# dropbox/lepton

Hardware: AMD Instinct MI355X
Metric: encode+decode MB/s (JPEG bytes/sec), bit-exact round trip (higher is better)
Workload: dtype int16/u8 (integer coder, no floating point)

## Files before the change

### lepton_amd/csrc/lep_enc5.h

```cpp
#pragma once
#include "lep_v3.h"
#ifdef LEP5_DEBUG
#include <cstdio>
#endif

namespace lep5 {
using namespace lep3;

constexpr int kRows = 64, kClasses = 10;
constexpr int kPRows = 63 + 14;
constexpr int kStreams = 2 * kRows * kClasses;
WDEV int stream_id(int ci, int row, int k) { return (ci * kRows + row) * kClasses + k; }
constexpr int kCoefSlice = 12 * 11 + 10 + 1;
constexpr int kSignSlice = 48, kNzSlice = 6 * 32, kEdgeNzSlice = 8 * 12, kDcSlice = 17 * 11 + 10 + 1;
constexpr uint32_t kThreshWords = 2u * 256 * 8 * 128;

WDEV uint32_t coef_entry(uint32_t vlow, int nres, int len, int bsr, int k, int u) {
    return vlow | ((uint32_t)nres << 10) | ((uint32_t)len << 14) | ((uint32_t)bsr << 18) | ((uint32_t)k << 23) | ((uint32_t)u << 27);
}
WDEV int coef_units(int len, int nres) { return ((len < 11 ? len + 1 : 11) + nres + 3) >> 2; }
WDEV uint32_t thresh_entry(uint32_t tbits, int n, int pcls, int lt, int u) {
    return tbits | ((uint32_t)n << 10) | ((uint32_t)pcls << 14) | ((uint32_t)lt << 23) | ((uint32_t)u << 27);
}
constexpr int kKeyRec = 4, kNzRec = 8, kEnRec = 8, kDcRec = 24;
// ... 1353 lines not shown
        LEP5_XSYNC();
        if (MODE == kEmit && wave == 0) {
            LANES(l) if (l < 16) LEP5_WSH(this).cursor[stream_id(l >> 3, 63, l & 7)] = LEP5_WSH(this).tcur[l];
            LSYNC();
            LANES(l) {
                for (int i = l; i < kStreams; i += 64)
                    for (uint32_t j = LEP5_WSH(this).cursor[i]; j < pl->base[i + 1]; ++j) gst(units() + j, 0u);
            }
        }
        return 0;
    }
};


constexpr int kCountWords = kStreams + 5;
WDEV void plan_segment(const uint32_t* counts, SegPlan5* P) {
    uint32_t at = 0;
    for (int i = 0; i < kStreams; ++i) { P->base[i] = at; P->cnt[i] = counts[i]; at += (counts[i] + 3u) & ~3u; }
    P->base[kStreams] = at;
    uint32_t bytes = at * 4;
    P->sign_cnt[0] = counts[kStreams]; P->sign_cnt[1] = counts[kStreams + 1];
    P->sign_base[0] = bytes; bytes += (P->sign_cnt[0] + 15u) & ~15u;
    P->sign_base[1] = bytes; bytes += (P->sign_cnt[1] + 15u) & ~15u;
    P->nblocks = counts[kStreams + 2];
    P->key_base = bytes; bytes += ((P->nblocks * (uint32_t)kKeyRec) + 15u) & ~15u;
    P->nz_base = bytes; bytes += P->nblocks * (uint32_t)kNzRec;
    P->en_base = bytes; bytes += P->nblocks * (uint32_t)kEnRec;
    P->dc_base = bytes; bytes += P->nblocks * (uint32_t)kDcRec;
    P->cls_base = bytes; bytes += 2u * kNumCls * 4u;
    P->place_base = bytes; bytes += 4u * P->nblocks * 4u;
    bytes = (bytes + 15u) & ~15u;
    P->nzs_base = bytes; bytes += (P->nblocks + 4u * 20u) * (uint32_t)kNzRec;
    P->ens_base[0] = bytes; bytes += (P->nblocks + 4u * 16u) * 4u;
    P->ens_base[1] = bytes; bytes += (P->nblocks + 4u * 16u) * 4u;
    P->dcs_base = bytes; bytes += (P->nblocks + 4u * 12u) * (uint32_t)kDcRec;
    bytes = (bytes + 15u) & ~15u;
    P->ckpt_base = bytes; bytes += (uint32_t)(kMaxParts * sizeof(Ckpt5));
    P->wstate_base = bytes; bytes += 64u;
    bytes = (bytes + 255u) & ~255u;
    P->ntiles = counts[kStreams + 4];
    P->at_base = bytes; bytes += P->ntiles * (uint32_t)(kAtRows * 64 * 4);
    P->arena_bytes = (bytes + 255u) & ~255u;
    P->bins_cap = (counts[kStreams + 3] + 127u) & ~127u;
    P->nbins = 0; P->status = 0; P->arena_off = 0; P->bins_off = 0;
}
template <class W>
WDEV void export_counts(const W& w, const Walk5Shared* sh, uint32_t* counts) {
    LANES(l) {
        for (int i = l; i < kStreams; i += 64) counts[i] = sh->cursor[i];
        if (l == 0) { counts[kStreams] = w.sign_pos[0]; counts[kStreams + 1] = w.sign_pos[1]; counts[kStreams + 2] = w.ord0; counts[kStreams + 3] = w.nbins; counts[kStreams + 4] = w.tile_no; }
    }
}

}
```

### lepton_amd/csrc/lep_gpu.hip

```cpp
#include <hip/hip_runtime.h>

#include <algorithm>
#include <cstdio>
#include <cstdlib>
#include <cstring>
#include <mutex>
#include <string>
#include <vector>

#include "../../include/lepton_mi355x.h"
#include "lep_buffers.h"

#define LEP_DEV __device__ __forceinline__
#include "lep_core.h"
#include "lep_enc3.h"
#include "lep_dec4.h"
#include "lep_enc5.h"
#include "lep_huff.h"
#include "lep_huffdec.h"
#include "lep_huffdec_simt.h"
#include "lep_huff_simt.h"
#include "lep_huffprog.h"
#include "lep_huffprog_simt.h"
#include "lep_huffprogdec.h"
// ... 89 lines not shown
        if (d >= 2) {
            const lep4::DivBy m = lep4::DivBy::of((uint32_t)d);
            const int32_t k = (int32_t)(0x7fffffff / d);
            for (int32_t n : {0, 1, -1, d, d - 1, -d, -d + 1, k * d, k * d - 1, -(k * d), 0x7fffffff, (int32_t)0x80000000, (int32_t)(f * 0x01000193u ^ t * 0x9e3779b9u)})
                if (lep4::div_by(n, m.mul, m.shift) != n / d) atomicAdd(mismatches, 1u);
        }
    }
}

template <int WAVES, int SCMASK = LEP_DEC4_SCALAR>
__global__ __launch_bounds__(64, WAVES) void lep_decode_v4_kernel(const ImageDev* __restrict__ images, const SegDev* __restrict__ segs,
                                                           uint32_t* models, NSum* ns_area, const uint64_t* ns_offsets,
                                                           uint8_t* streams, uint32_t* stream_len, int32_t* status, uint32_t* bins) {
    __shared__ lep4::Dec4Shared sh;
    const int s = blockIdx.x, lane = threadIdx.x;
    const SegDev seg = segs[s];
    const ImageDev* img = images + seg.image;
    uint32_t* model = models + (size_t)s * kModelStride;
    NSum* ns = ns_area + ns_offsets[s];
    reset_segment_state<lep3::kModelWords>(model, ns, img->ns_total, lane);
    __syncthreads();
    lep4::Dec4WaveT<SCMASK> w;
#ifdef LEP_PROF
    w.prof_begin(&g_prof4[s & 8191][0]);
#endif
    int rc = w.run(img, seg, model, ns, &sh, streams + seg.stream_off, stream_len[seg.slot]);
#ifdef LEP_PROF
    w.prof_end();
#endif
    if (lane != 0) return;
    status[seg.slot] = rc;
    bins[seg.slot] = w.nbins;
}


template <int MODE, int NW>
__global__ __launch_bounds__(64 * NW) void lep_enc5_walk_kernel(const ImageDev* __restrict__ images, const SegDev* __restrict__ segs, NSum* ns_all,
                                                         const uint64_t* __restrict__ ns_off, lep5::SegPlan5* plans, uint8_t* arena, uint16_t* bins,
                                                         uint32_t* counts, int part, int nparts) {
    lep5::Walk5Shared* sh = reinterpret_cast<lep5::Walk5Shared*>(lep5::lep5_lds);
    const int s = blockIdx.x;
    const SegDev seg = segs[s];
    lep5::SegPlan5* P = plans + s;
    if (MODE == lep5::kGather && P->status) return;
    lep5::Walk5<MODE, NW> w;
    const int rc = w.run(images + seg.image, seg, ns_all + ns_off[s], sh, P, arena, bins, (int)(threadIdx.x >> 6), part, nparts);
    if (threadIdx.x >= 64) return;
    if (MODE == lep5::kCount) lep5::export_counts(w, sh, counts + (size_t)s * lep5::kCountWords);
    if (threadIdx.x == 0) {
        if (MODE == lep5::kEmit) P->status = rc;
        if (MODE == lep5::kGather && part + 1 == nparts) P->nbins = w.nbins;
    }
}
template <int PHASE>
__global__ __launch_bounds__(64) void lep_enc5_wchunk_kernel(const lep5::SegPlan5* __restrict__ plans, const uint16_t* __restrict__ bins, const SegDev* __restrict__ segs,
                                                         int nseg, int K, lep5::WChunk5* recs, uint8_t* streams, uint32_t* stream_len, int32_t* status, uint32_t* nbins_out) {
    const int id = (int)(blockIdx.x * 64 + threadIdx.x);
    if (PHASE == 0 || PHASE == 2) {
        const int seg = id / K, k = id - seg * K;
        if (seg >= nseg) return;
        if (PHASE == 2) __builtin_amdgcn_s_setprio(3);
        if (PHASE == 0) lep5::wchunk_range_lane(plans[seg], bins, recs + (size_t)seg * K + k, k, K);
        else lep5::wchunk_code_lane(plans[seg], bins, segs[seg], streams, recs + (size_t)seg * K + k, k, K);
    } else {
        if (id >= nseg) return;
        if (PHASE == 1) { status[segs[id].slot] = 0; nbins_out[segs[id].slot] = plans[id].nbins; lep5::wchunk_link_lane(plans[id], bins, recs + (size_t)id * K, K); }
        else lep5::wchunk_stitch_lane(plans[id], segs[id], streams, stream_len, status, recs + (size_t)id * K, K);
    }
}
__global__ void lep_enc5_plan_kernel(const uint32_t* __restrict__ counts, lep5::SegPlan5* plans, int nseg) {
    const int s = (int)(blockIdx.x * blockDim.x + threadIdx.x);
    if (s < nseg) lep5::plan_segment(counts + (size_t)s * lep5::kCountWords, plans + s);
}
__global__ __launch_bounds__(64) void lep_enc5_offsets_kernel(lep5::SegPlan5* plans, int nseg, uint64_t* totals) {
    uint64_t a = 0, b = 0;
    for (int s0 = 0; s0 < nseg; s0 += 64) {
        const int s = s0 + (int)threadIdx.x;
        const uint32_t ab = s < nseg ? plans[s].arena_bytes : 0u, bc = s < nseg ? plans[s].bins_cap : 0u;
        int oa, ob;
        const int va = (int)(ab >> 8), vb = (int)(bc >> 7);
        const int ta = lepwave::wave_excl_scan(&va, &oa), tb = lepwave::wave_excl_scan(&vb, &ob);
        if (s < nseg) { plans[s].arena_off = a + ((uint64_t)(uint32_t)oa << 8); plans[s].bins_off = b + ((uint64_t)(uint32_t)ob << 7); }
        a += (uint64_t)(uint32_t)ta << 8; b += (uint64_t)(uint32_t)tb << 7;
    }
    if (threadIdx.x == 0) { totals[0] = a; totals[1] = b; }
}
__global__ void lep_enc5_fill_kernel(uint4* p, size_t n16, uint32_t v) {
    const uint4 x = make_uint4(v, v, v, v);
    for (size_t i = blockIdx.x * (size_t)blockDim.x + threadIdx.x; i < n16; i += (size_t)gridDim.x * blockDim.x) p[i] = x;
}
__global__ __launch_bounds__(64) void lep_enc5_bucket_kernel(const lep5::SegPlan5* __restrict__ plans, uint8_t* arena) {
    __shared__ lep5::BucketShared sh;
    lep5::bucket_wave(plans + blockIdx.x, arena, &sh);
}
struct Fold5CoefShared { uint16_t slice[lep5::kCoefSlice * 64]; };
__global__ __launch_bounds__(64) void lep_enc5_fold_coef_kernel(const lep5::SegPlan5* __restrict__ plans, uint8_t* arena, int nseg, int groups) {
    __shared__ Fold5CoefShared shc;
    const int grp = (int)blockIdx.x % groups, job = (int)blockIdx.x / groups;
    const int ci = job / 630, row = (job % 630) / 10, k = job % 10;
    const int sid = lep5::stream_id(ci, row, k), seg = grp * 64 + (int)threadIdx.x;
    const bool work = seg < nseg && !plans[seg].status && plans[seg].cnt[sid] != 0;
    if (!__ballot(work)) return;
    lep5::fold_coef_wave(plans, arena, grp * 64, nseg, sid, reinterpret_cast<lep5::FoldShared*>(&shc));
}
struct Fold5SmallShared { uint16_t slice[lep5::kEdgeNzSlice * 64]; };
__global__ __launch_bounds__(64) void lep_enc5_fold_small_kernel(const lep5::SegPlan5* __restrict__ plans, uint8_t* arena, uint32_t* thresh_models, int nseg, int groups, int job0) {
// ... 172 lines not shown
    w.run_scan<true>(scans + k, &sh, rows, deps + k, progress, k);
}

__global__ __launch_bounds__(64, 8) void lep_huffman_decode_kernel(const lephuff::HuffDecImage* __restrict__ images, lephuff::HuffDecRow* rows) {
    __shared__ lephuff::HuffDecShared sh;
    __builtin_amdgcn_s_setprio(3);
    lephuff::HuffDecWave w;
    w.run(images + blockIdx.x, &sh, rows);
}

__global__ __launch_bounds__(64) void lep_huffman_simt_settle_kernel(const lephuff::HuffDecImage* __restrict__ images, lephuff::SimtImage* si, const lephuff::SimtWave* waves,
                                                                     const lephuff::SimtSub* in, lephuff::SimtSub* out, int settle) {
    __shared__ lephuff::SimtShared sh;
    const lephuff::SimtWave w = waves[blockIdx.x];
    lephuff::simt_guess_or_settle(images + w.image, &sh, si + w.image, in + si[w.image].first, out + si[w.image].first, w.first_sub, settle);
}
__global__ __launch_bounds__(64) void lep_huffman_simt_place_kernel(const lephuff::HuffDecImage* __restrict__ images, lephuff::SimtImage* si, const lephuff::SimtSub* sub,
                                                                    lephuff::SimtPlace* place, int passes, lephuff::HuffDecRow* rows) {
    const int i = (int)blockIdx.x;
    lephuff::simt_place(images + i, si + i, sub + si[i].first, place + si[i].first, passes, rows);
}
__global__ __launch_bounds__(64) void lep_huffman_simt_write_kernel(const lephuff::HuffDecImage* __restrict__ images, lephuff::SimtImage* si, const lephuff::SimtWave* waves,
                                                                    const lephuff::SimtSub* sub, const lephuff::SimtPlace* place, lephuff::HuffDecRow* rows) {
    __shared__ lephuff::SimtShared sh;
    __shared__ lephuff::SimtTile tile;
    const lephuff::SimtWave w = waves[blockIdx.x];
    lephuff::simt_write(images + w.image, &sh, &tile, si + w.image, sub + si[w.image].first, place + si[w.image].first, rows, w.first_sub);
}
__global__ void lep_huffman_simt_finish_kernel(const lephuff::HuffDecImage* __restrict__ images, int nimg, lephuff::HuffDecRow* rows, const lephuff::SimtImage* si) {
    const int i = (int)(blockIdx.x * blockDim.x + threadIdx.x);
    if (i >= nimg) return;
    lephuff::HuffDecRow* last = rows + images[i].rows_off + images[i].mcuv;
    int status = si[i].status & 0x3fffff;
    if (last->aux == lephuff::kHuffDecRowUnwritten) { status |= 2; last->aux = 255; }
    if (images[i].flags & lephuff::kHuffDecRstTable) {
        const int pad = lephuff::simt_intervals_pad(si + i, &status);
        last->aux = pad | (status << 8);
        return;
    }
    last->aux = (last->aux & (255 | lephuff::kHuffDecRowTruncated)) | (status << 8);
}

}

struct lep_gpu {
    int device = 0;
    hipStream_t stream = nullptr;
    hipEvent_t ev0 = nullptr, ev1 = nullptr;
    bool timed = false;
    bool released = false;
    int enc5_min = 8;
    hipStream_t stream2 = nullptr, stream3 = nullptr;
    hipEvent_t ev_fork = nullptr, ev_join = nullptr, ev_join3 = nullptr;
    int huffprog_pipeline = 1;
    int huffprog_split = 0;
    int huffprogdec_rst = 1;
    uint32_t huffprogdec_rst_floor = lephuff::kRstPieceFloor;
    int huffprogdec_win = 1;
    int huffprog_simt = 1;
    int huffprog_simt_rst = 1;
    uint32_t huffprog_forms[4] = {0, 0, 0, 0};
    int huffenc_simt = 1;
    int simt_sub_bits = 0;
    int huffprog_pipeline_max = 16384;
    int enc5_waves = 2;
    int enc5_parts = 8;
    hipEvent_t ev_part[8] = {nullptr, nullptr, nullptr, nullptr, nullptr, nullptr, nullptr, nullptr};
    long enc5_wlanes = 131072;
    int enc5_wmaxseg = 4096;
    int enc5_wchunks = 64;
    int enc5_gather_wgs = 0;
    int enc5_fold_apart = 0;
    size_t enc5_scratch_max = ~(size_t)0;
    hipEvent_t ev_stage[8] = {nullptr, nullptr, nullptr, nullptr, nullptr, nullptr, nullptr, nullptr};
    int nstage = 0;
    int enc_waves = 0;
    int enc_pair_max = 1280;
    int dec_company = 0;
    int dec_waves = 0;
    std::string err;
    const char* last_kernel = "";
    struct Vmm {
        bool on = false;
        size_t chunk = (size_t)512 << 20;
        hipMemAllocationProp prop;
        hipMemAccessDesc access;
        std::vector<hipMemGenericAllocationHandle_t> pool;
        size_t mapped_total = 0, creates = 0, releases = 0;
    } vmm;
    enum Ws {
        W_ENC5_ENTRIES,
        W_ENC5_BINLIST,
        W_MODELS, W_MODELS_1,
        W_NS, W_NS_1,
        W_TRIMMED,
        W_META = W_TRIMMED, W_META_1,
        W_ENC5_PLANS,
        W_ENC5_WCHUNKS,
        W_BLOCKS, W_STREAMS, W_LENS,
        W_HUFF, W_HUFF_1,
        W_HUFFENC, W_HUFFENC_1,
        W_HUFFPROG, W_HUFFPROG_1,
        W_HUFFPROGSIMT, W_HUFFPROGSIMT_1,
        W_HUFFSEQ, W_HUFFSEQ_1,
        W_HUFFPROGDEC,
        W_HUFFPROGRST,
        W_HUFFDEC,
        W_HUFFPAR,
        W_COUNT
    };
    lepbuf::DevBuf<> ws[W_COUNT];
    int cur = 0;
    hipEvent_t ev_enc5_done = nullptr;
    uint32_t* d_bins = nullptr;
    std::vector<uint32_t> h_bins;
    struct Staging { void* host = nullptr; size_t cap = 0; hipEvent_t ev = nullptr; bool used = false; };
    Staging staging[16];
    int staging_next = 0;
    std::vector<void*> staging_retired;
    lepbuf::PinBuf<char> h_huffprog[2];
    int huffprog_turn = 0;
};

#define HIPCHK(g, call)                                                                        \
// ... 74 lines not shown
    const size_t old = b.mapped;
    while (b.mapped < want) {
        hipMemGenericAllocationHandle_t h;
        if (!V.pool.empty()) { h = V.pool.back(); V.pool.pop_back(); --V.creates; }
        else if (hipMemCreate(&h, V.chunk, &V.prop, 0) != hipSuccess) {
            (void)hipGetLastError();
            if (may_release) { may_release = false; release_idle_caches(g); if (!V.pool.empty()) continue; }
            {
                while (b.mapped > old) { b.mapped -= V.chunk; (void)hipMemUnmap(b.va + b.mapped, V.chunk); V.pool.push_back(b.chunks.back()); b.chunks.pop_back(); V.mapped_total -= V.chunk; }
                g->err = "hipMemCreate: out of device memory";
                return LEP_GPU_ERROR;
            }
        }
        ++V.creates;
        if (hipMemMap(b.va + b.mapped, V.chunk, 0, h, 0) != hipSuccess) { (void)hipGetLastError(); (void)hipMemRelease(h); g->err = "hipMemMap failed"; return LEP_GPU_ERROR; }
        b.chunks.push_back(h); b.mapped += V.chunk; V.mapped_total += V.chunk;
    }
    if (b.mapped > old) HIPCHK(g, hipMemSetAccess(b.va + old, b.mapped - old, &V.access, 1));
    w.set(b.va, b.mapped);
    return 0;
}
static int ensure(lep_gpu* g, Workspace& w, size_t need, bool may_release = true) {
    if (w.cap >= need) return 0;
    if (g->vmm.on && (need >= ((size_t)32 << 20) || w.v.va)) {
        if (!w.v.va) HIPCHK(g, w.release());
        return vmm_ensure(g, w, need, may_release);
    }
    hipError_t e = w.ensure(need, need / 8);
    if (e != hipSuccess && may_release) {
        (void)hipGetLastError();
        release_idle_caches(g);
        e = w.ensure(need);
    }
    if (e != hipSuccess) { g->err = std::string("hipMalloc: ") + hipGetErrorString(e); return LEP_GPU_ERROR; }
    return 0;
}

#include "lep_derive.h"


constexpr int kEnc5NoMemory = -1000;
static int launch_enc5(lep_gpu* g, const ImageDev* d_img, const SegDev* d_seg, const uint64_t* d_nsoff, int nseg, uint8_t* d_streams,
                       uint32_t* d_stream_len, int32_t* d_status, hipStream_t st) {
    Workspace &models = g->ws[lep_gpu::W_MODELS + g->cur], &ns = g->ws[lep_gpu::W_NS + g->cur];
    Workspace &ws_plans = g->ws[lep_gpu::W_ENC5_PLANS], &ws_entries = g->ws[lep_gpu::W_ENC5_ENTRIES], &ws_binlist = g->ws[lep_gpu::W_ENC5_BINLIST], &wchunks = g->ws[lep_gpu::W_ENC5_WCHUNKS];
    if (!g->stream2) {
        HIPCHK(g, hipEventCreateWithFlags(&g->ev_enc5_done, hipEventDisableTiming));
        for (auto& e : g->ev_part) HIPCHK(g, hipEventCreateWithFlags(&e, hipEventDisableTiming));
        HIPCHK(g, hipStreamCreateWithFlags(&g->stream2, hipStreamNonBlocking));
        HIPCHK(g, hipStreamCreateWithFlags(&g->stream3, hipStreamNonBlocking));
        HIPCHK(g, hipEventCreateWithFlags(&g->ev_fork, hipEventDisableTiming));
        HIPCHK(g, hipEventCreateWithFlags(&g->ev_join, hipEventDisableTiming));
        HIPCHK(g, hipEventCreateWithFlags(&g->ev_join3, hipEventDisableTiming));
        for (auto& e : g->ev_stage) HIPCHK(g, hipEventCreate(&e));
    }
    lepbuf::Layout L;
    L.add<lep5::SegPlan5>((size_t)nseg);
    const size_t o_counts = L.add<uint32_t>((size_t)nseg * lep5::kCountWords), o_tot = L.add<uint64_t>(2);
    HIPCHK(g, hipStreamWaitEvent(st, g->ev_enc5_done, 0));
    if (int rc = ensure(g, ws_plans, L.padded())) return rc;
    lep5::SegPlan5* plans = ws_plans.at<lep5::SegPlan5>(0);
    uint32_t* counts = ws_plans.at<uint32_t>(o_counts);
    uint64_t* d_tot = ws_plans.at<uint64_t>(o_tot);
    const int groups = (nseg + 63) / 64;
    g->nstage = 0;
    HIPCHK(g, hipEventRecord(g->ev_stage[0], st));
    const bool two = g->enc5_waves == 2;
    const int nparts = std::min(std::max(g->enc5_parts, 1), (int)lep5::kMaxParts);
    auto walk = [&](int mode, uint8_t* entries, uint16_t* binlist, int part = 0) {
        size_t lds = lep5::walk_lds_bytes(mode);
        if (mode == lep5::kGather && g->enc5_gather_wgs > 0) lds = std::max(lds, (size_t)(160 * 1024 / g->enc5_gather_wgs) & ~(size_t)255);
#define LEP_WALK(MODE, NW) hipLaunchKernelGGL((lep_enc5_walk_kernel<MODE, NW>), dim3(nseg), dim3(64 * NW), lds, st, d_img, d_seg, (NSum*)ns.p, d_nsoff, plans, entries, binlist, counts, part, nparts)
        if (mode == lep5::kCount) { if (two) LEP_WALK(lep5::kCount, 2); else LEP_WALK(lep5::kCount, 1); }
        else if (mode == lep5::kEmit) { if (two) LEP_WALK(lep5::kEmit, 2); else LEP_WALK(lep5::kEmit, 1); }
        else { if (two) LEP_WALK(lep5::kGather, 2); else LEP_WALK(lep5::kGather, 1); }
#undef LEP_WALK
    };
    walk(lep5::kCount, nullptr, nullptr);
    hipLaunchKernelGGL(lep_enc5_plan_kernel, dim3(groups), dim3(64), 0, st, (const uint32_t*)counts, plans, nseg);
    hipLaunchKernelGGL(lep_enc5_offsets_kernel, dim3(1), dim3(64), 0, st, plans, nseg, d_tot);
    hipLaunchKernelGGL(lep_enc5_fill_kernel, dim3(4096), dim3(256), 0, st, (uint4*)models.p, (size_t)nseg * lep5::kThreshWords / 4, kBranchInit);
    uint64_t tot[2] = {0, 0};
    HIPCHK(g, hipMemcpyAsync(tot, d_tot, sizeof tot, hipMemcpyDeviceToHost, st));
    HIPCHK(g, hipStreamSynchronize(st));
    if ((size_t)tot[0] + (size_t)tot[1] * 2 > g->enc5_scratch_max || ensure(g, ws_entries, (size_t)tot[0] + 256, false) || ensure(g, ws_binlist, (size_t)tot[1] * 2 + 256, false)) {
        (void)hipGetLastError();
        g->err.clear();
        static bool told = false;
        if (!told) { told = true; fprintf(stderr, "lepton-mi355x: no room for the split-phase encoder's scratch (%.1f GB for %d segments): single-kernel encoder\n", ((double)tot[0] + 2.0 * (double)tot[1]) / 1e9, nseg); }
        return kEnc5NoMemory;
    }
    {
        HIPCHK(g, hipEventRecord(g->ev_stage[1], st));
        walk(lep5::kEmit, (uint8_t*)ws_entries.p, nullptr);
        HIPCHK(g, hipEventRecord(g->ev_stage[2], st));
        hipLaunchKernelGGL(lep_enc5_bucket_kernel, dim3(nseg), dim3(64), 0, st, (const lep5::SegPlan5*)plans, (uint8_t*)ws_entries.p);
        HIPCHK(g, hipEventRecord(g->ev_fork, st));
        HIPCHK(g, hipStreamWaitEvent(g->stream2, g->ev_fork, 0));
        HIPCHK(g, hipStreamWaitEvent(g->stream3, g->ev_fork, 0));
        if (g->enc5_fold_apart) {
            const int small0[4] = {0, 2, 14, 46}, big0[3] = {0, 12, 32};
            for (int i = 0; i < 3; ++i)
                hipLaunchKernelGGL(lep_enc5_fold_small_kernel, dim3((unsigned)groups * (small0[i + 1] - small0[i])), dim3(64), 0, st, (const lep5::SegPlan5*)plans, (uint8_t*)ws_entries.p,
                                   (uint32_t*)models.p, nseg, groups, small0[i]);
            for (int i = 0; i < 2; ++i)
                hipLaunchKernelGGL(lep_enc5_fold_big_kernel, dim3((unsigned)groups * (big0[i + 1] - big0[i])), dim3(64), 0, st, (const lep5::SegPlan5*)plans, (uint8_t*)ws_entries.p, nseg, groups, big0[i]);
        } else {
        hipLaunchKernelGGL(lep_enc5_fold_small_kernel, dim3((unsigned)groups * kFold5SmallJobs), dim3(64), 0, g->stream2, (const lep5::SegPlan5*)plans, (uint8_t*)ws_entries.p,
                           (uint32_t*)models.p, nseg, groups, 0);
        hipLaunchKernelGGL(lep_enc5_fold_big_kernel, dim3((unsigned)groups * kFold5BigJobs), dim3(64), 0, g->stream3, (const lep5::SegPlan5*)plans, (uint8_t*)ws_entries.p, nseg, groups, 0);
        }
        hipLaunchKernelGGL(lep_enc5_fold_coef_kernel, dim3((unsigned)groups * 1260u), dim3(64), 0, st, (const lep5::SegPlan5*)plans, (uint8_t*)ws_entries.p, nseg, groups);
        HIPCHK(g, hipEventRecord(g->ev_join, g->stream2));
        HIPCHK(g, hipEventRecord(g->ev_join3, g->stream3));
        HIPCHK(g, hipStreamWaitEvent(st, g->ev_join, 0));
        HIPCHK(g, hipStreamWaitEvent(st, g->ev_join3, 0));
        HIPCHK(g, hipEventRecord(g->ev_stage[3], st));
        int K = 0;
        if (g->enc5_wchunks >= 2 && nseg <= g->enc5_wmaxseg) { K = 1; while (K * 2 <= g->enc5_wchunks && (long)nseg * K * 2 <= g->enc5_wlanes) K *= 2; }
        if (K >= 2 && ensure(g, wchunks, (size_t)nseg * K * sizeof(lep5::WChunk5) + 256, false)) { (void)hipGetLastError(); g->err.clear(); K = 0; }
        if (K >= 2) {
            for (int part = 0; part < nparts; ++part) walk(lep5::kGather, (uint8_t*)ws_entries.p, (uint16_t*)ws_binlist.p, part);
            HIPCHK(g, hipEventRecord(g->ev_stage[4], st));
            lep5::WChunk5* recs = (lep5::WChunk5*)wchunks.p;
            const int lane_groups = (int)(((long)nseg * K + 63) / 64);
#define LEP_WCHUNK(PHASE, GRID) hipLaunchKernelGGL((lep_enc5_wchunk_kernel<PHASE>), dim3(GRID), dim3(64), 0, st, (const lep5::SegPlan5*)plans, (const uint16_t*)ws_binlist.p, d_seg, nseg, K, recs, d_streams, d_stream_len, d_status, g->d_bins)
            LEP_WCHUNK(0, lane_groups); LEP_WCHUNK(1, groups); LEP_WCHUNK(2, lane_groups); LEP_WCHUNK(3, groups);
#undef LEP_WCHUNK
            HIPCHK(g, hipEventRecord(g->ev_stage[5], st));
            g->nstage = 5;
        } else {
        for (int part = 0; part < nparts; ++part) {
            walk(lep5::kGather, (uint8_t*)ws_entries.p, (uint16_t*)ws_binlist.p, part);
            HIPCHK(g, hipEventRecord(g->ev_part[part], st));
            HIPCHK(g, hipStreamWaitEvent(g->stream2, g->ev_part[part], 0));
            hipLaunchKernelGGL(lep_enc5_write_kernel, dim3(groups), dim3(64), 0, g->stream2, (const lep5::SegPlan5*)plans, (const uint16_t*)ws_binlist.p, d_seg, nseg, d_streams,
                               d_stream_len, d_status, g->d_bins, (uint8_t*)ws_entries.p, part, nparts);
        }
        HIPCHK(g, hipEventRecord(g->ev_stage[4], st));
        HIPCHK(g, hipEventRecord(g->ev_join, g->stream2));
        HIPCHK(g, hipStreamWaitEvent(st, g->ev_join, 0));
        HIPCHK(g, hipEventRecord(g->ev_stage[5], st));
        g->nstage = 5;
        }
    }
    HIPCHK(g, hipEventRecord(g->ev_enc5_done, st));
    HIPCHK(g, hipGetLastError());
    g->last_kernel = "lep_enc5 (count | emit | fold | gather | write)";
    return 0;
}

static int upload(lep_gpu* g, void* dst, const void* src, size_t n, hipStream_t st) {
    if (!n) return 0;
// ... 115 lines not shown
            if (rc && rc != kEnc5NoMemory) return rc;
            done = rc == 0;
        }
        if (done) {}
        else if (waves == 2) {
            g->last_kernel = "lep_encode_v3x2_kernel";
            hipLaunchKernelGGL(lep_encode_v3x2_kernel, dim3(nseg), dim3(128), 0, st, (const ImageDev*)(meta + o_img),
                               (const SegDev*)(meta + o_seg), (uint32_t*)models.p, (NSum*)ns.p, (const uint64_t*)(meta + o_ns),
                               d_streams, d_stream_len, d_status, g->d_bins);
        }
        else if (waves >= 8) { g->last_kernel = "lep_encode_v3_kernel<8>"; LEP_LAUNCH_ENC3(8); }
        else { g->last_kernel = "lep_encode_v3_kernel<4>"; LEP_LAUNCH_ENC3(4); }
#undef LEP_LAUNCH_ENC3
    }
    HIPCHK(g, hipGetLastError());
    HIPCHK(g, hipEventRecord(g->ev1, st));
    g->timed = true;
    return 0;
}

__attribute__((constructor)) static void lep_runtime_defaults() { setenv("GPU_MAX_HW_QUEUES", "8", 0); }

extern "C" {

static std::mutex g_live_mu;
static std::vector<lep_gpu*> g_live;
static bool g_exit_hook = false;
static void release_device_side(lep_gpu* g);
static void release_all_at_exit() {
    std::lock_guard<std::mutex> lk(g_live_mu);
    for (lep_gpu* g : g_live) release_device_side(g);
    g_live.clear();
}

int lep_gpu_create(int device, lep_gpu** out) {
    lep_gpu* g = new lep_gpu;
    g->device = device;
    if (const char* e = getenv("LEP_DEC_WAVES")) g->dec_waves = atoi(e) == 4 ? 4 : (atoi(e) == 8 ? 8 : 0);
    if (const char* e = getenv("LEP_ENC_WAVES")) g->enc_waves = atoi(e) == 4 ? 4 : (atoi(e) == 8 ? 8 : (atoi(e) == 2 ? 2 : 0));
    if (const char* e = getenv("LEP_ENC_PAIR_MAX")) g->enc_pair_max = atoi(e);
    if (const char* e = getenv("LEP_ENC5_MIN")) g->enc5_min = atoi(e);
    if (const char* e = getenv("LEP_HUFFPROG_PIPELINE")) g->huffprog_pipeline = atoi(e);
    if (const char* e = getenv("LEP_HUFFPROG_PIPELINE_MAX")) g->huffprog_pipeline_max = atoi(e);
    if (const char* e = getenv("LEP_HUFFDEC_SIMT_BITS")) g->simt_sub_bits = std::max(0, atoi(e));
    if (const char* e = getenv("LEP_HUFFENC_SIMT")) g->huffenc_simt = atoi(e) != 0;
    if (const char* e = getenv("LEP_HUFFPROG_SIMT")) g->huffprog_simt = atoi(e) != 0;
    if (const char* e = getenv("LEP_HUFFPROG_SIMT_RST")) g->huffprog_simt_rst = atoi(e) != 0;
    if (const char* e = getenv("LEP_HUFFPROGDEC_WIN")) g->huffprogdec_win = atoi(e) != 0;
    if (const char* e = getenv("LEP_HUFFPROGDEC_RST")) g->huffprogdec_rst = atoi(e) != 0;
    if (const char* e = getenv("LEP_HUFFPROGDEC_RST_FLOOR")) g->huffprogdec_rst_floor = (uint32_t)std::max(1, atoi(e));
    if (const char* e = getenv("LEP_HUFFPROG_SPLIT")) g->huffprog_split = atoi(e) != 0;
    if (const char* e = getenv("LEP_ENC5_WAVES")) g->enc5_waves = atoi(e) == 1 ? 1 : 2;
    if (const char* e = getenv("LEP_ENC5_FOLD_APART")) g->enc5_fold_apart = atoi(e);
    if (const char* e = getenv("LEP_ENC5_GATHER_WGS")) g->enc5_gather_wgs = atoi(e);
    if (const char* e = getenv("LEP_ENC5_PARTS")) g->enc5_parts = atoi(e);
    if (const char* e = getenv("LEP_ENC5_WCHUNKS")) g->enc5_wchunks = atoi(e);
    if (const char* e = getenv("LEP_ENC5_WLANES")) g->enc5_wlanes = atol(e);
    if (const char* e = getenv("LEP_ENC5_WMAXSEG")) g->enc5_wmaxseg = atoi(e);
    if (const char* e = getenv("LEP_ENC5_SCRATCH_MAX")) g->enc5_scratch_max = (size_t)strtoull(e, nullptr, 10);
    int n = 0;
    if (hipGetDeviceCount(&n) != hipSuccess || n <= device) { delete g; return LEP_GPU_ERROR; }
    if (hipSetDevice(device) != hipSuccess || hipStreamCreate(&g->stream) != hipSuccess ||
        hipEventCreate(&g->ev0) != hipSuccess || hipEventCreate(&g->ev1) != hipSuccess) { delete g; return LEP_GPU_ERROR; }
    vmm_init(g);
    {
        std::lock_guard<std::mutex> lk(g_live_mu);
        g_live.push_back(g);
        if (!g_exit_hook) { g_exit_hook = true; atexit(release_all_at_exit); }
    }
    *out = g;
    return 0;
}

static void release_device_side(lep_gpu* g) {
    if (g->released) return;
    g->released = true;
    (void)hipSetDevice(g->device);
    (void)hipStreamSynchronize(g->stream);
    if (g->ev_enc5_done) (void)hipEventDestroy(g->ev_enc5_done);
    for (auto& e : g->ev_part) if (e) (void)hipEventDestroy(e);
    for (auto& e : g->ev_stage) if (e) (void)hipEventDestroy(e);
    if (g->ev_fork) (void)hipEventDestroy(g->ev_fork);
    if (g->ev_join) (void)hipEventDestroy(g->ev_join);
    if (g->ev_join3) (void)hipEventDestroy(g->ev_join3);
    if (g->stream2) (void)hipStreamDestroy(g->stream2);
    if (g->stream3) (void)hipStreamDestroy(g->stream3);
    for (Workspace& w : g->ws) dev_release(g, w);
    vmm_destroy(g);
    if (g->ev0) (void)hipEventDestroy(g->ev0);
    if (g->ev1) (void)hipEventDestroy(g->ev1);
    if (g->stream) (void)hipStreamDestroy(g->stream);
    for (auto& h : g->h_huffprog) (void)h.release();
    for (lep_gpu::Staging& sl : g->staging) { if (sl.host) (void)hipHostFree(sl.host); if (sl.ev) (void)hipEventDestroy(sl.ev); sl = lep_gpu::Staging(); }
    for (void* p : g->staging_retired) (void)hipHostFree(p);
    g->staging_retired.clear();
}

void lep_gpu_destroy(lep_gpu* g) {
    if (!g) return;
    {
        std::lock_guard<std::mutex> lk(g_live_mu);
        for (size_t i = 0; i < g_live.size(); ++i) if (g_live[i] == g) { g_live.erase(g_live.begin() + i); break; }
        release_device_side(g);
    }
    delete g;
}

const char* lep_gpu_last_error(lep_gpu* g) { return g ? g->err.c_str() : "no gpu object"; }

int lep_gpu_encode_device(lep_gpu* g, const lep_image_desc* images, int nimg, const lep_segment* segs, int nseg,
                          uint8_t* d_streams, const uint64_t* stream_offsets, uint32_t* d_stream_len, int32_t* d_status,
                          void* hip_stream) {
    return launch<false>(g, images, nimg, segs, nseg, d_streams, stream_offsets, d_stream_len, d_status,
                         hip_stream ? (hipStream_t)hip_stream : g->stream);
}

int lep_gpu_decode_device(lep_gpu* g, const lep_image_desc* images, int nimg, const lep_segment* segs, int nseg,
                          const uint8_t* d_streams, const uint64_t* stream_offsets, const uint32_t* d_stream_len,
                          int32_t* d_status, void* hip_stream) {
    return launch<true>(g, images, nimg, segs, nseg, const_cast<uint8_t*>(d_streams), stream_offsets,
                        const_cast<uint32_t*>(d_stream_len), d_status, hip_stream ? (hipStream_t)hip_stream : g->stream);
}

static_assert(sizeof(lep_huff_image) == sizeof(lephuff::HuffImage) && sizeof(lep_huff_segment) == sizeof(lephuff::HuffSegment) &&
              sizeof(lep_huff_end) == sizeof(lephuff::HuffEnd) && sizeof(lep_huff_end) == 16, "C ABI mirrors");

int lep_gpu_huffman_encode_device(lep_gpu* g, const lep_huff_image* images, int nimg, const lep_huff_segment* segs, int nseg,
                                  uint8_t* d_out, uint32_t* d_out_len, lep_huff_end* d_ends, void* hip_stream) {
    if (!g) return LEP_GPU_ERROR;
    if (nseg <= 0) return 0;
    hipStream_t st = hip_stream ? (hipStream_t)hip_stream : g->stream;
    HIPCHK(g, hipSetDevice(g->device));
    lepbuf::Layout D;
    D.add<lep_huff_image>((size_t)nimg);
    const size_t o_seg = D.add<lep_huff_segment>((size_t)nseg);
    const int set = g->cur & 1;
    Workspace &huff = g->ws[lep_gpu::W_HUFF + set], &huffenc = g->ws[lep_gpu::W_HUFFENC + set];
// ... 605 lines not shown
```

Before: 1570.

## Split encoder count pass into many tile-range workgroups with atomic merges

Replaces the one-workgroup-per-segment count walk with a count kernel that splits each segment's tiles into R ranges across many workgroups. Each range accumulates per-stream histograms in LDS and merges them into global counts with atomics. The default mode uses a new ballot-based direct coefficient counter instead of the full walk. The model-fill kernel moves to a second stream so it can overlap the count and plan stages. The goal is to remove the serial per-segment bottleneck of the count phase, at the cost of redundant tile seeking per range, atomic traffic, and the risk that the new counting formula diverges from what the walk produces.

```diff
diff --git a/lepton_amd/csrc/lep_enc5.h b/lepton_amd/csrc/lep_enc5.h
--- a/lepton_amd/csrc/lep_enc5.h
+++ b/lepton_amd/csrc/lep_enc5.h
@@ -1429,4 +1429,150 @@
     }
 }
 
-}
+typedef Walk5<kCount, 1> CountWalk5;
+struct Count5Shared { uint32_t hist[kStreams]; };
+#if LEP_ON_GPU
+#define LEP5_CSH(p) (*reinterpret_cast<lep5::Count5Shared*>(lep5::lep5_lds))
+#else
+#define LEP5_CSH(p) (*(p))
+#endif
+WDEV void count_add(uint32_t* p, uint32_t v) {
+#if LEP_ON_GPU
+    __hip_atomic_fetch_add(p, v, __ATOMIC_RELAXED, __HIP_MEMORY_SCOPE_AGENT);
+#else
+    *p += v;
+#endif
+}
+WDEV uint32_t segment_tiles(const ImageDev* image, const SegDev& seg, NSum* ns) {
+    CountWalk5::TileIter it;
+    CountWalk5::TileDesc t;
+    it.init(image, seg, ns);
+    uint32_t n = 0;
+    while (it.next(&t)) { n += (uint32_t)(it.row_blocks + 63) >> 6; it.row_x0 = it.row_blocks; }
+    return n;
+}
+WDEV bool seek_tile(CountWalk5::TileIter& it, uint32_t first, CountWalk5::TileDesc* t) {
+    uint32_t at = 0;
+    while (it.next(t)) {
+        const uint32_t in_row = (uint32_t)(it.row_blocks + 63) >> 6;
+        if (first - at < in_row) {
+            for (; at < first; ++at) it.next(t);
+            return true;
+        }
+        at += in_row;
+        it.row_x0 = it.row_blocks;
+    }
+    return false;
+}
+WDEV void count_flush(const uint32_t* hist, const uint32_t* sign_pos, uint32_t blocks, uint32_t nbins, uint32_t ntiles, int r, uint32_t* counts) {
+    LANES(l) {
+        for (int i = l; i < kStreams; i += 64) { const uint32_t c = hist[i]; if (c) count_add(counts + i, c); }
+        if (l == 0) {
+            if (sign_pos[0]) count_add(counts + kStreams, sign_pos[0]);
+            if (sign_pos[1]) count_add(counts + kStreams + 1, sign_pos[1]);
+            if (blocks) count_add(counts + kStreams + 2, blocks);
+            if (nbins) count_add(counts + kStreams + 3, nbins);
+            if (r == 0 && ntiles) count_add(counts + kStreams + 4, ntiles);
+        }
+    }
+}
+
+WDEV void count_range_blocks(const ImageDev* image, const SegDev& seg, NSum* ns, Walk5Shared* shared, int r, int R, uint32_t* counts) {
+    CountWalk5 w;
+    w.img = image; w.sh = shared; w.plan = nullptr; w.status = 0; w.wave = 0; w.arena = nullptr; w.bins = nullptr; w.AT = nullptr;
+    w.ord0 = 0; w.sign_pos[0] = w.sign_pos[1] = 0; w.nbins = 0; w.tile_no = 0; w.comp = -1; w.ci = 0;
+    LANES(l) for (int i = l; i < kStreams; i += 64) LEP5_WSH(&w).cursor[i] = 0u;
+    LSYNC();
+    const uint32_t ntiles = segment_tiles(image, seg, ns);
+    const uint32_t first = part_first_tile(ntiles, r, R), end = part_first_tile(ntiles, r + 1, R);
+    CountWalk5::TileIter it;
+    CountWalk5::TileDesc cur_t{}, nxt_t{};
+    LV(CountWalk5::TileRegs, regs);
+    it.init(image, seg, ns);
+    bool have = first < end && seek_tile(it, first, &cur_t);
+    if (have) w.fetch_tile(cur_t, regs);
+    for (uint32_t tno = first; have; ++tno) {
+        w.store_tile(cur_t, regs);
+        const bool more = tno + 1 < end && it.next(&nxt_t);
+        if (more) w.fetch_tile(nxt_t, regs);
+        w.tile(cur_t.x0, cur_t.nb, false, nullptr, nullptr);
+        cur_t = nxt_t;
+        have = more;
+    }
+    LSYNC();
+    count_flush(LEP5_WSH(&w).cursor, w.sign_pos, w.ord0, w.nbins, ntiles, r, counts);
+}
+
+WDEV void count_range_coefs(const ImageDev* image, const SegDev& seg, NSum* ns, Count5Shared* shared, int r, int R, uint32_t* counts) {
+    constexpr int kU = 8;
+    constexpr uint64_t kInterior = (1ull << 49) - 1;
+    (void)shared;
+    LV(uint64_t, behind);
+    LV(int, row); LV(int, coord); LV(int, thr); LV(int, lbins);
+    LANES(l) {
+        const uint64_t region = l < 49 ? kInterior : (l == 49 ? 0ull : (l < 57 ? 0x7full << 50 : 0x7full << 57));
+        L(behind) = region & ~((1ull << l) - 1);
+        L(row) = l < 49 ? l : l - 1;
+        L(coord) = l < 50 ? 0 : (l < 57 ? l - 49 : (l - 56) * 8);
+        L(thr) = 64; L(lbins) = 0;
+        for (int i = l; i < kStreams; i += 64) LEP5_CSH(shared).hist[i] = 0u;
+    }
+    LSYNC();
+    const uint32_t ntiles = segment_tiles(image, seg, ns);
+    const uint32_t first = part_first_tile(ntiles, r, R), end = part_first_tile(ntiles, r + 1, R);
+    CountWalk5::TileIter it;
+    CountWalk5::TileDesc t{};
+    it.init(image, seg, ns);
+    bool have = first < end && seek_tile(it, first, &t);
+    uint32_t sign_pos[2] = {0, 0}, blocks = 0, sbins = 0;
+    int comp = -1, ci = 0;
+    for (uint32_t tno = first; have; ++tno) {
+        if (t.comp != comp) {
+            comp = t.comp; ci = comp ? 1 : 0;
+            LANES(l) L(thr) = l >= 50 ? (int)image->min_thresh[comp][L(coord)] : 64;
+        }
+        const int16_t* src = t.row + (int64_t)t.x0 * 64;
+        for (int b0 = 0; b0 < t.nb; b0 += kU) {
+            struct Cf { int16_t v[kU]; };
+            LV(Cf, cf);
+            LANES(l) {
+#pragma unroll
+                for (int u = 0; u < kU; ++u) L(cf).v[u] = b0 + u < t.nb ? gld(src + (b0 + u) * 64 + l) : (int16_t)0;
+            }
+#pragma unroll
+            for (int u = 0; u < kU; ++u) {
+                if (b0 + u >= t.nb) break;
+                LV(int, nzp);
+                LANES(l) L(nzp) = L(cf).v[u] != 0;
+                const uint64_t m = lepwave::wave_ballot(nzp);
+                LANES(l) {
+                    const int v = iabs(L(cf).v[u]), len = bitlen((uint32_t)v), lc = len > 11 ? 11 : len;
+                    const int left = lepwave::popc64(m & L(behind));
+                    if (left > 0) {
+                        int nres = lc > 1 ? lc - 1 : 0;
+                        if (lc > 1 && lc - 2 >= L(thr)) {
+                            const int lt = imin(lc - L(thr), 7), un = (lc - 1 - L(thr) + 3) >> 2;
+                            lds_add(&LEP5_CSH(shared).hist[stream_id(ci, 63, lt)], (uint32_t)un);
+                            nres = L(thr);
+                        }
+                        const int k = l < 49 ? nzbin5(left) : left;
+                        lds_add(&LEP5_CSH(shared).hist[stream_id(ci, L(row), k)], (uint32_t)coef_units(lc, nres));
+                    }
+                    if (v && l != 49) L(lbins) += (lc < 11 ? lc + 1 : 11) + lc;
+                }
+                const uint64_t i7 = m & kInterior;
+                const uint32_t eh = (uint32_t)(m >> 50) & 127u, ev = (uint32_t)(m >> 57) & 127u;
+                const int n7 = lepwave::popc64(i7), nh = lepwave::popc64(eh), nv = lepwave::popc64(ev);
+                sign_pos[ci] += (uint32_t)(n7 + nh + nv + 1);
+                sbins += (uint32_t)((i7 ? 64 - __builtin_clzll(i7) : 0) - n7 + bitlen(eh) - nh + bitlen(ev) - nv + 12 + 22);
+            }
+        }
+        blocks += (uint32_t)t.nb;
+        have = tno + 1 < end && it.next(&t);
+    }
+    LSYNC();
+    const uint32_t nbins = sbins + (uint32_t)lepwave::wave_sum(lbins);
+    count_flush(LEP5_CSH(shared).hist, sign_pos, blocks, nbins, ntiles, r, counts);
+}
+
+}
diff --git a/lepton_amd/csrc/lep_gpu.hip b/lepton_amd/csrc/lep_gpu.hip
--- a/lepton_amd/csrc/lep_gpu.hip
+++ b/lepton_amd/csrc/lep_gpu.hip
@@ -165,6 +165,15 @@
         if (MODE == lep5::kGather && part + 1 == nparts) P->nbins = w.nbins;
     }
 }
+template <int MAP>
+__global__ __launch_bounds__(64) void lep_enc5_count_kernel(const ImageDev* __restrict__ images, const SegDev* __restrict__ segs, NSum* ns_all,
+                                                          const uint64_t* __restrict__ ns_off, uint32_t* counts, int R) {
+    const int s = (int)blockIdx.x / R, r = (int)blockIdx.x - s * R;
+    const SegDev seg = segs[s];
+    uint32_t* mine = counts + (size_t)s * lep5::kCountWords;
+    if (MAP == 1) lep5::count_range_blocks(images + seg.image, seg, ns_all + ns_off[s], reinterpret_cast<lep5::Walk5Shared*>(lep5::lep5_lds), r, R, mine);
+    else lep5::count_range_coefs(images + seg.image, seg, ns_all + ns_off[s], reinterpret_cast<lep5::Count5Shared*>(lep5::lep5_lds), r, R, mine);
+}
 template <int PHASE>
 __global__ __launch_bounds__(64) void lep_enc5_wchunk_kernel(const lep5::SegPlan5* __restrict__ plans, const uint16_t* __restrict__ bins, const SegDev* __restrict__ segs,
                                                          int nseg, int K, lep5::WChunk5* recs, uint8_t* streams, uint32_t* stream_len, int32_t* status, uint32_t* nbins_out) {
@@ -443,6 +452,7 @@
     int enc5_min = 8;
     hipStream_t stream2 = nullptr, stream3 = nullptr;
     hipEvent_t ev_fork = nullptr, ev_join = nullptr, ev_join3 = nullptr;
+    hipEvent_t ev_fill_go = nullptr, ev_fill_done = nullptr;
     int huffprog_pipeline = 1;
     int huffprog_split = 0;
     int huffprogdec_rst = 1;
@@ -461,6 +471,8 @@
     int enc5_wmaxseg = 4096;
     int enc5_wchunks = 64;
     int enc5_gather_wgs = 0;
+    int enc5_count = 2;
+    long enc5_count_wgs = 32768;
     int enc5_fold_apart = 0;
     size_t enc5_scratch_max = ~(size_t)0;
     hipEvent_t ev_stage[8] = {nullptr, nullptr, nullptr, nullptr, nullptr, nullptr, nullptr, nullptr};
@@ -641,6 +653,8 @@
         HIPCHK(g, hipEventCreateWithFlags(&g->ev_fork, hipEventDisableTiming));
         HIPCHK(g, hipEventCreateWithFlags(&g->ev_join, hipEventDisableTiming));
         HIPCHK(g, hipEventCreateWithFlags(&g->ev_join3, hipEventDisableTiming));
+        HIPCHK(g, hipEventCreateWithFlags(&g->ev_fill_go, hipEventDisableTiming));
+        HIPCHK(g, hipEventCreateWithFlags(&g->ev_fill_done, hipEventDisableTiming));
         for (auto& e : g->ev_stage) HIPCHK(g, hipEventCreate(&e));
     }
     lepbuf::Layout L;
@@ -660,15 +674,24 @@
         size_t lds = lep5::walk_lds_bytes(mode);
         if (mode == lep5::kGather && g->enc5_gather_wgs > 0) lds = std::max(lds, (size_t)(160 * 1024 / g->enc5_gather_wgs) & ~(size_t)255);
 #define LEP_WALK(MODE, NW) hipLaunchKernelGGL((lep_enc5_walk_kernel<MODE, NW>), dim3(nseg), dim3(64 * NW), lds, st, d_img, d_seg, (NSum*)ns.p, d_nsoff, plans, entries, binlist, counts, part, nparts)
-        if (mode == lep5::kCount) { if (two) LEP_WALK(lep5::kCount, 2); else LEP_WALK(lep5::kCount, 1); }
-        else if (mode == lep5::kEmit) { if (two) LEP_WALK(lep5::kEmit, 2); else LEP_WALK(lep5::kEmit, 1); }
+        if (mode == lep5::kEmit) { if (two) LEP_WALK(lep5::kEmit, 2); else LEP_WALK(lep5::kEmit, 1); }
         else { if (two) LEP_WALK(lep5::kGather, 2); else LEP_WALK(lep5::kGather, 1); }
 #undef LEP_WALK
     };
-    walk(lep5::kCount, nullptr, nullptr);
+    HIPCHK(g, hipEventRecord(g->ev_fill_go, st));
+    HIPCHK(g, hipStreamWaitEvent(g->stream2, g->ev_fill_go, 0));
+    hipLaunchKernelGGL(lep_enc5_fill_kernel, dim3(4096), dim3(256), 0, g->stream2, (uint4*)models.p, (size_t)nseg * lep5::kThreshWords / 4, kBranchInit);
+    HIPCHK(g, hipEventRecord(g->ev_fill_done, g->stream2));
+    {
+        const int R = (int)std::min<long>(std::max<long>((g->enc5_count_wgs + nseg - 1) / nseg, 1), 64);
+        HIPCHK(g, hipMemsetAsync(counts, 0, (size_t)nseg * lep5::kCountWords * sizeof(uint32_t), st));
+        if (g->enc5_count == 1)
+            hipLaunchKernelGGL((lep_enc5_count_kernel<1>), dim3((unsigned)nseg * (unsigned)R), dim3(64), lep5::kWalkLdsCount, st, d_img, d_seg, (NSum*)ns.p, d_nsoff, counts, R);
+        else
+            hipLaunchKernelGGL((lep_enc5_count_kernel<2>), dim3((unsigned)nseg * (unsigned)R), dim3(64), sizeof(lep5::Count5Shared), st, d_img, d_seg, (NSum*)ns.p, d_nsoff, counts, R);
+    }
     hipLaunchKernelGGL(lep_enc5_plan_kernel, dim3(groups), dim3(64), 0, st, (const uint32_t*)counts, plans, nseg);
     hipLaunchKernelGGL(lep_enc5_offsets_kernel, dim3(1), dim3(64), 0, st, plans, nseg, d_tot);
-    hipLaunchKernelGGL(lep_enc5_fill_kernel, dim3(4096), dim3(256), 0, st, (uint4*)models.p, (size_t)nseg * lep5::kThreshWords / 4, kBranchInit);
     uint64_t tot[2] = {0, 0};
     HIPCHK(g, hipMemcpyAsync(tot, d_tot, sizeof tot, hipMemcpyDeviceToHost, st));
     HIPCHK(g, hipStreamSynchronize(st));
@@ -677,6 +700,7 @@
         g->err.clear();
         static bool told = false;
         if (!told) { told = true; fprintf(stderr, "lepton-mi355x: no room for the split-phase encoder's scratch (%.1f GB for %d segments): single-kernel encoder\n", ((double)tot[0] + 2.0 * (double)tot[1]) / 1e9, nseg); }
+        HIPCHK(g, hipStreamWaitEvent(st, g->ev_fill_done, 0));
         return kEnc5NoMemory;
     }
     {
@@ -688,6 +712,7 @@
         HIPCHK(g, hipStreamWaitEvent(g->stream2, g->ev_fork, 0));
         HIPCHK(g, hipStreamWaitEvent(g->stream3, g->ev_fork, 0));
         if (g->enc5_fold_apart) {
+            HIPCHK(g, hipStreamWaitEvent(st, g->ev_fill_done, 0));
             const int small0[4] = {0, 2, 14, 46}, big0[3] = {0, 12, 32};
             for (int i = 0; i < 3; ++i)
                 hipLaunchKernelGGL(lep_enc5_fold_small_kernel, dim3((unsigned)groups * (small0[i + 1] - small0[i])), dim3(64), 0, st, (const lep5::SegPlan5*)plans, (uint8_t*)ws_entries.p,
@@ -909,6 +934,8 @@
     if (const char* e = getenv("LEP_HUFFPROG_SPLIT")) g->huffprog_split = atoi(e) != 0;
     if (const char* e = getenv("LEP_ENC5_WAVES")) g->enc5_waves = atoi(e) == 1 ? 1 : 2;
     if (const char* e = getenv("LEP_ENC5_FOLD_APART")) g->enc5_fold_apart = atoi(e);
+    if (const char* e = getenv("LEP_ENC5_COUNT")) g->enc5_count = atoi(e) == 1 ? 1 : 2;
+    if (const char* e = getenv("LEP_ENC5_COUNT_WGS")) g->enc5_count_wgs = atol(e);
     if (const char* e = getenv("LEP_ENC5_GATHER_WGS")) g->enc5_gather_wgs = atoi(e);
     if (const char* e = getenv("LEP_ENC5_PARTS")) g->enc5_parts = atoi(e);
     if (const char* e = getenv("LEP_ENC5_WCHUNKS")) g->enc5_wchunks = atoi(e);
@@ -940,6 +967,8 @@
     if (g->ev_fork) (void)hipEventDestroy(g->ev_fork);
     if (g->ev_join) (void)hipEventDestroy(g->ev_join);
     if (g->ev_join3) (void)hipEventDestroy(g->ev_join3);
+    if (g->ev_fill_go) (void)hipEventDestroy(g->ev_fill_go);
+    if (g->ev_fill_done) (void)hipEventDestroy(g->ev_fill_done);
     if (g->stream2) (void)hipStreamDestroy(g->stream2);
     if (g->stream3) (void)hipStreamDestroy(g->stream3);
     for (Workspace& w : g->ws) dev_release(g, w);
```

New measurement: 1573 (median of 6 runs). No clear change (+0.2%).
